# EasyVision-Ton/VMG

Measured on AMD Instinct MI355X. Metric: LR-frames/s (train: forward+loss+backward+AdamW), VMG-REDS-few_levels 4x SR, higher is better.
Workload: dtype bf16; 1 GPU; VMG-REDS-few_levels train step, per-GPU batch 4x7x3x64x64 -> 4x SR (BASELINE configs[1]); global_batch=4, frames_per_clip=7, parallelism=dp1, launch=eager, recompute_chains=False, fp8_chains=False

## Files before the change

include/vmg_hip.h:

```cpp
#ifndef VMG_HIP_H
#define VMG_HIP_H

#include <stdint.h>

#ifdef __cplusplus
extern "C" {
#endif

#define VMG_F32 0
#define VMG_BF16 1

#define VMG_ACT_NONE 0
#define VMG_ACT_RELU 1
#define VMG_ACT_LRELU 2
#define VMG_ACT_GELU 3

#define VMG_CONV_GENERAL 0
#define VMG_CONV_KSPLIT 2
#define VMG_CONV_WS 3
#define VMG_CONV_LINEAR_WRES 4
#define VMG_CONV_WSTAT 6

const char* vmg_last_error(void);
int vmg_version(void);

typedef struct vmg_ctx vmg_ctx;
vmg_ctx* vmg_create(int device);
int vmg_destroy(vmg_ctx* ctx);
int vmg_ctx_device(const vmg_ctx* ctx);
int vmg_max_lds_bytes(void);

int64_t vmg_conv_pack_bytes(int dtype, int ks, int on, int nsrc, const int* src_ch, int cout_tiles);
int vmg_conv_pack(int dtype, const float* w, int O, int I, int ks, int o0, int on, int nsrc, const int* src_off,
                  const int* src_ch, int transpose_flip, int cout_tiles, void* packed, void* stream);

int64_t vmg_convws_pack_bytes(int on, int nsrc, const int* src_ch, int cout_tiles);
int vmg_convws_pack(const float* w, int O, int I, int o0, int on, int nsrc, const int* src_off, const int* src_ch, int transpose_flip,
                    int cout_tiles, void* packed, void* stream);

typedef struct vmg_conv_desc {
  int dtype, ks, cout_tiles;
  int N, H, W, Cout;
  int nsrc;
  const void* src[4];
  int64_t src_ps[4];
  int src_ch[4];
  const void* packed;
  const float* bias;
  void* out;
  int64_t out_ps;
  void* out_pre;
  const void* res;
  int64_t res_ps;
  const void* aux;
  int64_t aux_ps;
  int act;
  float slope, alpha;
  int actgrad;
  int pixel_shuffle;
  int mt;
  int deep;
} vmg_conv_desc;

int vmg_conv_fwd(const vmg_conv_desc* d, void* stream);
enum {
  VMG_CONV_FAM_IGEMM = 1,
  VMG_CONV_FAM_KSPLIT = 2,
  VMG_CONV_FAM_WS = 3,
  VMG_CONV_FAM_LINEAR_WRES = 4,
  VMG_CONV_FAM_WSTAT = 5,
  VMG_CONV_PLAN_INTS = 11
};
int vmg_conv_fwd_plan(const vmg_conv_desc* d, int ncu, int* plan);
typedef struct vmg_chain_desc {
  int dtype, N, H, W, C, nblk, nsrc;
  const void* src[4];
  int64_t src_ps[4];
  int src_ch[4];
  const void* packed0;
  const float* bias0;
  float slope0;
  int cout_tiles0, deep0;
  const void* const* packed1;
  const float* const* bias1;
  const void* const* packed2;
  const float* const* bias2;
  float r_scaling;
  int cout_tiles, deep;
  void* const* y;
  void* const* t;
  void* const* g_y;
  void* const* g_t;
} vmg_chain_desc;
int vmg_resblock_chain_fwd(const vmg_chain_desc* d, void* stream);
int vmg_resblock_chain_bwd(const vmg_chain_desc* d, void* stream);

void* vmg_replay_build(void* hip_graph, int* n_ops, int* n_kernels);
int vmg_replay_kernel_info(void* replay, int idx, void** func, unsigned* grid_x, unsigned* block_x, void** first_arg);
int vmg_replay_run(void* replay, int first, int last, void* stream);
void vmg_replay_destroy(void* replay);

int vmg_pack_entry_bytes(void);
int vmg_pack_entry(void* entry, int kind, int dtype, const float* w, int O, int I, int ks, int o0, int on, int nsrc, const int* src_off,
// ... 280 lines not shown
```

vmg_amd/csrc/common.h:

```cpp
#pragma once
#include <hip/hip_runtime.h>
#include <stdint.h>
#include <stdio.h>
#include <string.h>

#include "../../include/vmg_hip.h"

typedef __bf16 bf16;
typedef __attribute__((ext_vector_type(8))) __bf16 bf16x8;
typedef __attribute__((ext_vector_type(4))) __bf16 bf16x4;
typedef __attribute__((ext_vector_type(4))) float f32x4;

#define LDS_PTR(p) ((__attribute__((address_space(3))) void*)(p))
#define GLB_PTR(p) ((const __attribute__((address_space(1))) void*)(p))

void vmg_set_error(const char* fmt, ...);

constexpr int VMG_MAX_DEVICES = 64;
int vmg_current_device();
int vmg_cu_count(int device);

bool vmg_prof_before(int klass, long long pixels, hipStream_t st);
void vmg_prof_after(hipStream_t st);
#define VMG_PROF_CONV3X3 1
// ... 30 lines not shown
  static constexpr int CHUNKB = 32;
};

__device__ __forceinline__ float to_f32(bf16 v) { return (float)v; }
__device__ __forceinline__ float to_f32(float v) { return v; }
template <typename T>
__device__ __forceinline__ T from_f32(float v);
template <>
__device__ __forceinline__ bf16 from_f32<bf16>(float v) { return (bf16)v; }
template <>
__device__ __forceinline__ float from_f32<float>(float v) { return v; }

__device__ __forceinline__ void load4(const bf16* p, float v[4]) {
  bf16x4 t = *reinterpret_cast<const bf16x4*>(p);
  v[0] = (float)t[0]; v[1] = (float)t[1]; v[2] = (float)t[2]; v[3] = (float)t[3];
}
__device__ __forceinline__ void load4(const float* p, float v[4]) {
  float4 t = *reinterpret_cast<const float4*>(p);
  v[0] = t.x; v[1] = t.y; v[2] = t.z; v[3] = t.w;
}
__device__ __forceinline__ void store4(bf16* p, const float v[4]) {
  bf16x4 t = {(bf16)v[0], (bf16)v[1], (bf16)v[2], (bf16)v[3]};
  *reinterpret_cast<bf16x4*>(p) = t;
}
__device__ __forceinline__ void store4(float* p, const float v[4]) {
  *reinterpret_cast<float4*>(p) = make_float4(v[0], v[1], v[2], v[3]);
}

__device__ __forceinline__ float gelu_erf(float x) { return 0.5f * x * (1.0f + erff(x * 0.70710678118654752440f)); }
__device__ __forceinline__ float gelu_erf_grad(float x) {
  return 0.5f * (1.0f + erff(x * 0.70710678118654752440f)) + x * __expf(-0.5f * x * x) * 0.39894228040143267794f;
}

__device__ __forceinline__ float wave_sum(float v) {
#pragma unroll
  for (int o = 32; o > 0; o >>= 1) v += __shfl_xor(v, o, 64);
  return v;
}
__device__ __forceinline__ float wave_max(float v) {
#pragma unroll
  for (int o = 32; o > 0; o >>= 1) v = fmaxf(v, __shfl_xor(v, o, 64));
  return v;
}

static inline int64_t cdiv64(int64_t a, int64_t b) { return (a + b - 1) / b; }
static inline int cdiv(int a, int b) { return (a + b - 1) / b; }
```

vmg_amd/csrc/conv_igemm.hip:

```cpp
#include <stdlib.h>

#include <type_traits>

#include "common.h"

namespace {

constexpr int MAX_ISRC = 32;
constexpr int CBMAX = 160;

__host__ __device__ constexpr int kstg(int ks) { return ks > 1 ? ks : 2; }
__host__ __device__ constexpr int stage_bytes(int ks, int ntb, int cb) { return kstg(ks) * 4 * ntb * 16 * cb; }
__host__ __device__ constexpr int stage_stride(int ks, int ntb, int cb) { return (stage_bytes(ks, ntb, cb) + 4095) / 4096 * 4096; }
__host__ __device__ inline int stages_of(int ks, int ch) {
  const int nb = (ch / 8 + 3) / 4;
  return ks > 1 ? ks * nb : (nb + 1) / 2;
}

struct ConvK {
  const char* src[MAX_ISRC];
  long long src_ps[MAX_ISRC];
  short src_ch[MAX_ISRC];
  short src_nst[MAX_ISRC];
  int src_pixb[MAX_ISRC];
// ... 410 lines not shown
  for (int mt = 0; mt < MT; ++mt) {
    f32x4 r[NTB];
#pragma unroll
    for (int ct = 0; ct < NTB; ++ct) r[ct] = acc[ct][mt];
    conv_epilogue_row<T, KS, NTB>(a, r, wave * MT + mt, TH, cb, nt_real, n, ty, tx, m0, px, g);
  }
}

template <int NTB>
struct EpiLds {
  static constexpr int COB = NTB * 16, C8 = 2 * NTB, PSTR = COB * 4 + 16, NIT = (16 * C8 + 63) / 64;
  static constexpr int BYTES = 16 * PSTR;
};

template <int KS, int NTB>
__device__ __forceinline__ void conv_epilogue_prefetch8(const ConvK& a, int row, int TH, int cb, int n, int ty, int tx, long long m0, int lane,
                                                        bf16x8 (&pre_res)[EpiLds<NTB>::NIT], bf16x8 (&pre_aux)[EpiLds<NTB>::NIT]) {
  using E = EpiLds<NTB>;
  const bf16* res = reinterpret_cast<const bf16*>(a.res);
  const bf16* aux = reinterpret_cast<const bf16*>(a.aux);
#pragma unroll
  for (int it = 0; it < E::NIT; ++it) {
    const int j = it * 64 + lane, pxi = j / E::C8, c8 = j - pxi * E::C8;
    long long pix;
    const bool valid = conv_row_pixel<KS>(a, row, TH, n, ty, tx, m0, pxi & 15, pix);
    const int co = cb * E::COB + c8 * 8;
    if (j < 16 * E::C8 && valid && co < a.Cout) {
      if (res) pre_res[it] = *reinterpret_cast<const bf16x8*>(res + pix * a.res_ps + co);
      if (aux) pre_aux[it] = *reinterpret_cast<const bf16x8*>(aux + pix * a.aux_ps + co);
    }
  }
}

template <int KS, int NTB>
__device__ __forceinline__ void conv_epilogue_lds8(const ConvK& a, const f32x4 (&acc)[NTB], char* stg, int row, int TH, int cb, int n, int ty, int tx,
                                                   long long m0, int lane, const bf16x8 (&pre_res)[EpiLds<NTB>::NIT],
                                                   const bf16x8 (&pre_aux)[EpiLds<NTB>::NIT], const float* lbias) {
  using E = EpiLds<NTB>;
  const int px = lane & 15, g = lane >> 4;
#pragma unroll
  for (int ct = 0; ct < NTB; ++ct) *reinterpret_cast<f32x4*>(stg + px * E::PSTR + (ct * 16 + g * 4) * 4) = acc[ct];
  bf16* out = reinterpret_cast<bf16*>(a.out);
  bf16* out_pre = reinterpret_cast<bf16*>(a.out_pre);
  const float neg = a.act == VMG_ACT_RELU ? 0.f : (a.act == VMG_ACT_LRELU ? a.slope : 1.f);
#pragma unroll
  for (int it = 0; it < E::NIT; ++it) {
    const int j = it * 64 + lane, pxi = j / E::C8, c8 = j - pxi * E::C8;
    long long pix;
    const bool valid = conv_row_pixel<KS>(a, row, TH, n, ty, tx, m0, pxi & 15, pix);
    const int co = cb * E::COB + c8 * 8;
    if (!(j < 16 * E::C8 && valid && co < a.Cout) || VMG_DBG(a, 8)) continue;
    const f32x4 lo = *reinterpret_cast<const f32x4*>(stg + pxi * E::PSTR + c8 * 32);
    const f32x4 hi = *reinterpret_cast<const f32x4*>(stg + pxi * E::PSTR + c8 * 32 + 16);
    float v[8] = {lo[0], lo[1], lo[2], lo[3], hi[0], hi[1], hi[2], hi[3]};
    if (a.bias) {
      const f32x4 b0 = *reinterpret_cast<const f32x4*>(lbias + c8 * 8), b1 = *reinterpret_cast<const f32x4*>(lbias + c8 * 8 + 4);
#pragma unroll
      for (int r = 0; r < 4; ++r) { v[r] += b0[r]; v[4 + r] += b1[r]; }
    }
    if (out_pre) {
      bf16x8 t;
#pragma unroll
      for (int r = 0; r < 8; ++r) t[r] = (bf16)v[r];
      *reinterpret_cast<bf16x8*>(out_pre + pix * a.out_ps + co) = t;
    }
    if (a.act == VMG_ACT_GELU) {
#pragma unroll
      for (int r = 0; r < 8; ++r) v[r] = gelu_erf(v[r]) * a.alpha;
    } else {
#pragma unroll
      for (int r = 0; r < 8; ++r) v[r] = (v[r] > 0.f ? v[r] : v[r] * neg) * a.alpha;
    }
    if (a.aux) {
#pragma unroll
      for (int r = 0; r < 8; ++r) {
        const float u = (float)pre_aux[it][r];
        v[r] *= a.actgrad == 3 ? gelu_erf_grad(u) : (u > 0.f ? 1.f : (a.actgrad == 2 ? a.slope : 0.f));
      }
    }
    if (a.res) {
#pragma unroll
      for (int r = 0; r < 8; ++r) v[r] += (float)pre_res[it][r];
    }
    bf16x8 t;
#pragma unroll
    for (int r = 0; r < 8; ++r) t[r] = (bf16)v[r];
    *reinterpret_cast<bf16x8*>(out + pix * a.out_ps + co) = t;
  }
}

template <typename T, int KS, int NTB>
__global__ __launch_bounds__(256, (NTB <= 3 ? 3 : 2)) void conv_ksplit_kernel(const ConvK a) {
  constexpr int ES = ElemTraits<T>::ES, CB = ElemTraits<T>::CHUNKB;
  constexpr int TH = 4;
  constexpr int TWH = 16 + KS - 1;
  constexpr int COB = NTB * 16;
  constexpr int SS = stage_stride(KS, NTB, CB);
  constexpr int KSB = 4 * COB * CB;
  extern __shared__ __attribute__((aligned(16))) char smem[];
  char* halo = smem;
  char* zslot = smem + a.halo_bytes;
  float* lbias = reinterpret_cast<float*>(zslot + 16);
  if (VMG_DBG(a, 16)) return;

  const int tid = threadIdx.x, lane = tid & 63;
  const int wave = __builtin_amdgcn_readfirstlane(tid >> 6);
  const int px = lane & 15, g = lane >> 4;
  const int cb = blockIdx.y;
  const int nt_real = min(NTB, (a.Cout - cb * COB + 15) >> 4);
  int n = 0, ty = 0, tx = 0;
// ... 210 lines not shown
    }
  };
  int boff[NK];
#pragma unroll
  for (int k = 0; k < NK; ++k) {
    const int sb = k / NKS, kk = k - sb * NKS;
    boff[k] = px * pixb + (sb * CH + min(4 * kk + g, CH - 1)) * CB;
  }

  issue(t0, 0);
  int buf = 0;
  for (int t = t0; t < t1; ++t, buf ^= 1) {
    const long long m0 = (long long)t * 16;
    bf16x8 pre_res[EpiLds<NTB>::NIT], pre_aux[EpiLds<NTB>::NIT];
    conv_epilogue_prefetch8<KS, NTB>(a, 0, 4, cb, 0, 0, 0, m0, lane, pre_res, pre_aux);
    if (t + 1 < t1) {
      issue(t + 1, buf ^ 1);
      asm volatile("s_waitcnt vmcnt(%0)" ::"n"(NDMA) : "memory");
    } else {
      asm volatile("s_waitcnt vmcnt(0)" ::: "memory");
    }
    f32x4 acc[NTB];
#pragma unroll
    for (int ct = 0; ct < NTB; ++ct) acc[ct] = f32x4{0.f, 0.f, 0.f, 0.f};
    const char* xb = xbuf + buf * XBUF;
#pragma unroll
    for (int k = 0; k < NK; ++k) {
      Frag<T> xf;
      xf.load(xb + boff[k]);
#pragma unroll
      for (int ct = 0; ct < NTB; ++ct) acc[ct] = mma(wres[k][ct], xf, acc[ct]);
    }
    conv_epilogue_lds8<KS, NTB>(a, acc, patch, 0, 4, cb, 0, 0, 0, m0, lane, pre_res, pre_aux, a.bias ? a.bias + cb * COB : nullptr);
  }
}

template <int NCT, int NB, bool FULL>
__global__ __launch_bounds__(512, 1) void conv_wstat_kernel(const ConvK a, int ntiles) {
  using T = bf16;
  constexpr int KS = 3, CB = 16, TH = 8, TWH = 18, THH = 10;
  constexpr int COB = NCT * 16, KSB = 4 * COB * CB;
  constexpr int SS = stage_stride(KS, NCT, CB);
  constexpr int NK = 9 * NB, RW = NCT < 2 ? NCT : 2;
  constexpr int PIXB = 144;
  constexpr int HVEC = THH * TWH * 9, NDMA = (HVEC + 63) / 64, HB = NDMA * 1024;
  constexpr int PSTR = COB * 4 + 16, C8 = 2 * NCT, NITEM = 128 * C8;
  extern __shared__ __attribute__((aligned(16))) char smem[];
  const int tid = threadIdx.x, lane = tid & 63;
  const int wave = __builtin_amdgcn_readfirstlane(tid >> 6);
  const int px = lane & 15, g = lane >> 4;
  const int cb = blockIdx.y;
  const int CH = a.src_ch[0] >> 3;
  constexpr int wbytes = 3 * NB * SS;
  char* wl = smem;
  char* halo = smem + wbytes;
  float* lbias = reinterpret_cast<float*>(halo + 2 * HB);
  char* patch = halo + 2 * HB + COB * 4;

  const int per_xcd = gridDim.x >> 3;
  const int xcd = blockIdx.x & 7, local = blockIdx.x >> 3;
  const int band = (ntiles + 7) >> 3;
  const int band0 = xcd * band, band1 = min(ntiles, band0 + band);
  auto tile_of = [&](int it) { return band0 + it * per_xcd + local; };
  auto barrier = [&]() {
    asm volatile("s_waitcnt lgkmcnt(0)" ::: "memory");
    __builtin_amdgcn_s_barrier();
// ... 829 lines not shown

int choose_pixb(int ch, int es, int cb) {
  static const int grp[4][16] = {{0, 1, 2, 3, 12, 13, 14, 15, 20, 21, 22, 23, 24, 25, 26, 27},
                                 {4, 5, 6, 7, 8, 9, 10, 11, 16, 17, 18, 19, 28, 29, 30, 31},
                                 {32, 33, 34, 35, 44, 45, 46, 47, 52, 53, 54, 55, 56, 57, 58, 59},
                                 {36, 37, 38, 39, 40, 41, 42, 43, 48, 49, 50, 51, 60, 61, 62, 63}};
  int best = ch * es, bestc = 1 << 30;
  for (int pad = 0; pad <= 240; pad += 16) {
    const int pixb = ch * es + pad;
    int worst = 0;
    for (int gi = 0; gi < 4; ++gi) {
      int cnt[16] = {0};
      for (int j = 0; j < 16; ++j) {
        const int l = grp[gi][j];
        const int addr = (l & 15) * pixb + (l >> 4) * cb;
        int c = ++cnt[(addr >> 4) & 15];
        if (c > worst) worst = c;
      }
    }
    if (worst < bestc) { bestc = worst; best = pixb; }
    if (worst == 1) break;
  }
  return best;
}

struct ConvPlan {
  int family;
  int dtype, ks, mt, ntb;
  int variant;
  int vec8;
  int gx, gy;
  int tpw;
  int lds;
};

constexpr int epi_lds_bytes(int ntb) { return 16 * (ntb * 16 * 4 + 16); }
constexpr int wres_lds_bytes(int ntb, int ns) { return 4 * (2 * 5 * ns * 1024 + ((epi_lds_bytes(ntb) + 1023) & ~1023)); }
constexpr int wstat_lds_bytes(int nct, int nb) {
  return 3 * nb * stage_stride(3, nct, 16) + 2 * (((10 * 18 * 9 + 63) / 64) * 1024) + nct * 16 * 4 + 128 * (nct * 64 + 16);
}
constexpr int ws_stage_bytes(int nct) { return 3 * nct * 16 * 64; }

template <typename T, int KS, int MT, int NTB>
int launch_conv(const ConvK& k, const ConvPlan& p, hipStream_t st) {
  const int lds = p.lds;
  auto fn = conv_igemm_kernel<T, KS, MT, NTB>;
  static bool attr_set[VMG_MAX_DEVICES] = {};
  const int dev = vmg_current_device();
  if (!attr_set[dev]) {
    (void)hipFuncSetAttribute(reinterpret_cast<const void*>(fn), hipFuncAttributeMaxDynamicSharedMemorySize, 160 * 1024);
    attr_set[dev] = true;
  }
  const bool prof = (KS == 3 && sizeof(T) == 2 && k.nsrc == 1 && k.src_ch[0] == 144 && k.Cout == 144) && vmg_prof_before(VMG_PROF_CONV3X3, k.M, st);
  hipLaunchKernelGGL(fn, dim3((unsigned)p.gx, p.gy), dim3(256), lds, st, k);
  if (prof) vmg_prof_after(st);
  VMG_LAUNCH_CHECK();
  return 0;
}

template <typename T, int KS, int MT>
int dispatch_ntb(const ConvK& k, const ConvPlan& p, hipStream_t st) {
  switch (p.ntb) {
    case 1: return launch_conv<T, KS, MT, 1>(k, p, st);
    case 3: return launch_conv<T, KS, MT, 3>(k, p, st);
    case 4: return launch_conv<T, KS, MT, 4>(k, p, st);
    case 5: return launch_conv<T, KS, MT, 5>(k, p, st);
    case 7: return launch_conv<T, KS, MT, 7>(k, p, st);
    case 8: return launch_conv<T, KS, MT, 8>(k, p, st);
    case 9: return launch_conv<T, KS, MT, 9>(k, p, st);
  }
  vmg_set_error("conv: cout_tiles must be 1, 3, 4, 5, 7, 8 or 9 (got %d)", p.ntb);
  return -1;
}

// ... 22 lines not shown
  hipLaunchKernelGGL(fn, dim3((unsigned)p.gx, p.gy), dim3(256), lds, st, k);
  if (prof) vmg_prof_after(st);
  VMG_LAUNCH_CHECK();
  return 0;
}

template <typename T, int KS>
int dispatch_ksplit(const ConvK& k, const ConvPlan& p, hipStream_t st) {
  switch (p.ntb) {
    case 1: return launch_ksplit<T, KS, 1>(k, p, st);
    case 3: return launch_ksplit<T, KS, 3>(k, p, st);
    case 4: return launch_ksplit<T, KS, 4>(k, p, st);
    case 5: return launch_ksplit<T, KS, 5>(k, p, st);
  }
  vmg_set_error("conv (k-split): cout_tiles must be 1, 3, 4 or 5 (got %d)", p.ntb);
  return -1;
}

template <int NTB, int NS = 1>
int launch_linear_wres(const ConvK& k, const ConvPlan& p, hipStream_t st) {
  static_assert(wres_lds_bytes(NTB, NS) == 4 * (2 * 5 * NS * 1024 + ((EpiLds<NTB>::BYTES + 1023) & ~1023)), "linear_wres_kernel: LDS");
  const int lds = p.lds;
  auto fn = linear_wres_kernel<NTB, NS>;
  static bool attr_set[VMG_MAX_DEVICES] = {};
  const int dev = vmg_current_device();
  if (!attr_set[dev]) {
    (void)hipFuncSetAttribute(reinterpret_cast<const void*>(fn), hipFuncAttributeMaxDynamicSharedMemorySize, 160 * 1024);
    attr_set[dev] = true;
  }
  hipLaunchKernelGGL(fn, dim3((unsigned)p.gx, p.gy), dim3(256), lds, st, k, (int)cdiv64(k.M, 16), p.tpw);
  VMG_LAUNCH_CHECK();
  return 0;
}

template <int NCT, int NB, bool FULL>
int launch_wstat2(const ConvK& k, const ConvPlan& p, hipStream_t st) {
  constexpr int lds = wstat_lds_bytes(NCT, NB);
  static_assert(lds <= 160 * 1024, "conv_wstat_kernel: LDS");
  auto fn = conv_wstat_kernel<NCT, NB, FULL>;
  static bool attr_set[VMG_MAX_DEVICES] = {};
  const int dev = vmg_current_device();
  if (!attr_set[dev]) {
    (void)hipFuncSetAttribute(reinterpret_cast<const void*>(fn), hipFuncAttributeMaxDynamicSharedMemorySize, 160 * 1024);
    attr_set[dev] = true;
  }
  hipLaunchKernelGGL(fn, dim3((unsigned)p.gx, p.gy), dim3(512), lds, st, k, (int)((long long)k.N * k.tiles_y * k.tiles_x));
  VMG_LAUNCH_CHECK();
  return 0;
}

template <int NCT, int NB>
int launch_wstat(const ConvK& k, const ConvPlan& p, hipStream_t st) {
  return (p.variant >> 4) ? launch_wstat2<NCT, NB, true>(k, p, st) : launch_wstat2<NCT, NB, false>(k, p, st);
}

template <int NCT>
int launch_ws(const ConvK& k, const ConvPlan& p, hipStream_t st) {
  using G = WsGeo<NCT>;
  static_assert(ws_stage_bytes(NCT) == G::STG, "conv_ws_kernel: stage bytes");
  const int lds = p.lds;
  auto fn = conv_ws_kernel<NCT>;
  static bool attr_set[VMG_MAX_DEVICES] = {};
  const int dev = vmg_current_device();
  if (!attr_set[dev]) {
    (void)hipFuncSetAttribute(reinterpret_cast<const void*>(fn), hipFuncAttributeMaxDynamicSharedMemorySize, 160 * 1024);
    attr_set[dev] = true;
// ... 171 lines not shown
  int rc;
  if (kind == 1) {
    VMG_CHECK(ks == 3 && dtype == VMG_BF16, "pack_entry: the weight-streaming layout is bf16 3x3");
    rc = fill_pack_ws(e.p, e.total, w, O, I, o0, on, nsrc, src_off, src_ch, transpose_flip, cout_tiles, packed);
  } else {
    rc = fill_pack_std(e.p, e.total, dtype, w, O, I, ks, o0, on, nsrc, src_off, src_ch, transpose_flip, cout_tiles, packed);
  }
  if (rc) return rc;
  e.kind = kind; e.dtype = dtype; e.blk0 = blk0;
  long long nb = e.p.fast3 ? (e.p.units + 255) / 256 : (e.total + 256LL * 16 - 1) / (256LL * 16);
  e.nblk = (int)(nb < 1 ? 1 : (nb > 64 ? 64 : nb));
  memcpy(entry, &e, sizeof(e));
  return e.nblk;
}

extern "C" int vmg_pack_run(const void* plan_dev, int n, int total_blocks, void* stream) {
  VMG_CHECK(plan_dev && n > 0 && total_blocks > 0, "pack_run: bad arguments");
  static_assert(sizeof(PackEntry) % 4 == 0, "the block-owner table sits behind the entries");
  hipLaunchKernelGGL(pack_batch_kernel, dim3(total_blocks), dim3(256), 0, (hipStream_t)stream, (const PackEntry*)plan_dev, n);
  VMG_LAUNCH_CHECK();
  return 0;
}

static int conv_plan(const vmg_conv_desc* d, int ncu, ConvK& k, ConvPlan& p) {
  VMG_CHECK(d != nullptr, "conv_fwd: null descriptor");
  VMG_CHECK(d->ks == 1 || d->ks == 3 || d->ks == 7, "conv_fwd: ks must be 1, 3 or 7");
  VMG_CHECK(d->dtype == VMG_F32 || d->dtype == VMG_BF16, "conv_fwd: bad dtype");
  VMG_CHECK(d->nsrc >= 1 && d->nsrc <= 4, "conv_fwd: nsrc must be 1..4");
  VMG_CHECK(d->N > 0 && d->H > 0 && d->W > 0 && d->Cout > 0, "conv_fwd: bad shape");
  VMG_CHECK(d->packed && d->out, "conv_fwd: null packed weights / output");
  VMG_CHECK(!d->pixel_shuffle || (d->Cout % 4 == 0), "conv_fwd: pixel_shuffle needs Cout %% 4 == 0");
  VMG_CHECK(!(d->actgrad != 0 && d->aux == nullptr), "conv_fwd: actgrad without aux");
  VMG_CHECK(d->deep == VMG_CONV_GENERAL || d->deep == VMG_CONV_KSPLIT || d->deep == VMG_CONV_WS || d->deep == VMG_CONV_LINEAR_WRES ||
                d->deep == VMG_CONV_WSTAT,
            "conv_fwd: unknown kernel route deep = %d", d->deep);
  const int es = d->dtype == VMG_BF16 ? 2 : 4, cbytes = es * 8;
  memset(&k, 0, sizeof(k));
  memset(&p, 0, sizeof(p));
  short xoff[MAX_ISRC];
  int parent[MAX_ISRC];
  const int n = expand_sources(d->nsrc, nullptr, d->src_ch, xoff, k.src_ch, parent);
  VMG_CHECK(n > 0, "conv_fwd: source channel counts must be multiples of 8");
  int mt = d->mt;
  if (d->dtype == VMG_F32) mt = 1;
  const long long M = (long long)d->N * d->H * d->W;
  const int ntb = d->cout_tiles;
  VMG_CHECK(ntb > 0, "conv_fwd: cout_tiles must be positive");
  const int ncb = cdiv(d->Cout, ntb * 16);
  if (d->ks == 7) mt = 1;
  if (mt == 0) mt = 1;
  VMG_CHECK(mt == 1 || mt == 2, "conv_fwd: mt must be 1 or 2");
  const int TH = 4 * mt, TWH = 16 + d->ks - 1, THH = TH + d->ks - 1;
  int kt = 0, halo = 0;
  for (int s = 0; s < n; ++s) {
    const int par = parent[s];
    VMG_CHECK(d->src[par] != nullptr, "conv_fwd: null source %d", par);
    VMG_CHECK(d->src_ps[par] >= d->src_ch[par] && (d->src_ps[par] * es) % 16 == 0, "conv_fwd: source pixel stride must be >= channels and 16-byte aligned");
    VMG_CHECK(((uintptr_t)d->src[par]) % 16 == 0, "conv_fwd: source pointer must be 16-byte aligned");
    k.src[s] = (const char*)d->src[par] + (long long)xoff[s] * es;
    k.src_ps[s] = d->src_ps[par];
    k.src_nst[s] = (short)stages_of(d->ks, k.src_ch[s]);
    k.src_pixb[s] = choose_pixb(k.src_ch[s], es, cbytes);
    kt += k.src_nst[s];
    const int hb = THH * TWH * k.src_pixb[s];
    if (hb > halo) halo = hb;
  }
  k.nsrc = n;
// ... 26 lines not shown
    int kt3 = 0, halo3 = 0;
    for (int s = 0; s < n; ++s) {
      k.src_pixb[s] = k.src_ch[s] * 2;
      k.src_nst[s] = (short)(ws_ksteps(k.src_ch[s] >> 3) / 3);
      kt3 += k.src_nst[s];
      const int hb = 10 * 18 * k.src_pixb[s];
      if (hb > halo3) halo3 = hb;
    }
    k.nstages = kt3;
    k.halo_bytes = (halo3 + 1023) & ~1023;
    k.tiles_y = cdiv(d->H, 8);
    k.ring = ntb <= 3 ? 3 : ((k.halo_bytes + 4 * ws_stage_bytes(ntb) + ntb * 16 * 4 <= 160 * 1024) ? 4 : 3);
    p.lds = k.halo_bytes + k.ring * ws_stage_bytes(ntb) + ntb * 16 * 4;
    VMG_CHECK(p.lds <= 160 * 1024, "conv (weight-streaming): LDS request %d B exceeds 160 KiB", p.lds);
    const long long nblk = (long long)k.N * k.tiles_y * k.tiles_x;
    VMG_CHECK(nblk > 0 && nblk < (1ll << 31), "conv: bad grid %lld", nblk);
    p.family = VMG_CONV_FAM_WS; p.gx = (int)nblk;
    return 0;
  }
  if (d->deep == VMG_CONV_WSTAT && d->dtype == VMG_BF16 && d->ks == 3 && mt == 1 && k.vec8 && n == 1 && (ntb == 1 || ntb == 3 || ntb == 4) && k.src_ch[0] <= 64 && k.src_ch[0] % 8 == 0 &&
      k.src_ps[0] % 8 == 0 && d->W <= 255 * 16 && (long long)d->W * k.src_ps[0] * 2 * 10 < (1ll << 31)) {
    const int nb = (k.src_ch[0] / 8 + 3) / 4;
    VMG_CHECK(k.nstages == 3 * nb, "conv (weights-stationary): %d stages in the pack, %d expected", k.nstages, 3 * nb);
    k.tiles_y = cdiv(d->H, 8);
    const long long ntiles = (long long)k.N * k.tiles_y * k.tiles_x;
    VMG_CHECK(ntiles > 0 && ntiles < (1ll << 30), "conv: bad tile count %lld", ntiles);
    int nwg = cus() & ~7;
    if (nwg < 8) nwg = 8;
    while (nwg > 8 && (long long)(nwg >> 3) > cdiv64(ntiles, 8)) nwg -= 8;
    const bool full = k.res || k.aux || k.out_pre || k.act == VMG_ACT_GELU;
    p.family = VMG_CONV_FAM_WSTAT; p.variant = nb | (full ? 16 : 0); p.gx = nwg; p.lds = wstat_lds_bytes(ntb, nb);
    return 0;
  }
  if (d->deep == VMG_CONV_LINEAR_WRES && d->dtype == VMG_BF16 && d->ks == 1 && k.vec8 && (ntb == 3 || ntb == 5)) {
    int ns = 0;
    if (n == 1 && k.src_ch[0] <= 160 && k.src_pixb[0] == k.src_ch[0] * 2) ns = 1;
    else if (n == 2 && ntb == 3 && d->nsrc == 1 && k.src_ch[0] == k.src_ch[1] && k.src_ch[0] <= 160 && k.src[1] == k.src[0] + k.src_ch[0] * 2 &&
             k.src_nst[0] == k.src_nst[1])
      ns = 2;
    if (ns) {
      const long long ntiles = cdiv64(k.M, 16);
      VMG_CHECK(ntiles > 0 && ntiles < (1ll << 31), "conv: bad tile count %lld", ntiles);
      const int wg_per_cu = ns == 1 ? 2 : 1, c = cus();
      long long waves = (long long)(wg_per_cu * c / ncb > 0 ? wg_per_cu * c / ncb : 1) * 4;
      long long tpw = cdiv64(ntiles, waves);
      if (tpw < 4) tpw = 4;
      p.family = VMG_CONV_FAM_LINEAR_WRES; p.variant = ns; p.gx = (int)cdiv64(cdiv64(ntiles, tpw), 4); p.tpw = (int)tpw; p.lds = wres_lds_bytes(ntb, ns);
      return 0;
    }
  }
  const bool ksplit = d->ks != 7 && d->deep == VMG_CONV_KSPLIT;
  if (ksplit) {
    VMG_CHECK(d->dtype == VMG_BF16 && mt == 1, "conv_fwd: the k-split variant is bf16, mt = 1");
    if (!(ntb == 1 || ntb == 3 || ntb == 4 || ntb == 5)) {
      vmg_set_error("conv (k-split): cout_tiles must be 1, 3, 4 or 5 (got %d)", ntb);
      return -1;
    }
    const int scratch = 12 * ntb * 1024;
    p.lds = (k.halo_bytes > scratch ? k.halo_bytes : scratch) + 16 + ntb * 16 * 4;
    VMG_CHECK(p.lds <= 160 * 1024, "conv (k-split): LDS request %d B exceeds 160 KiB", p.lds);
    k.halo_bytes = p.lds - 16 - ntb * 16 * 4;
    p.family = VMG_CONV_FAM_KSPLIT;
  } else {
    if (d->ks == 7) {
      if (!(ntb == 1 || ntb == 2 || ntb == 4)) {
        vmg_set_error("conv (7x7): cout_tiles must be 1, 2 or 4 (got %d)", ntb);
        return -1;
      }
    } else if (!(ntb == 1 || ntb == 3 || ntb == 4 || ntb == 5 || ntb == 7 || ntb == 8 || ntb == 9)) {
      vmg_set_error("conv: cout_tiles must be 1, 3, 4, 5, 7, 8 or 9 (got %d)", ntb);
      return -1;
    }
    p.lds = k.halo_bytes + 2 * stage_stride(d->ks, ntb, cbytes);
    VMG_CHECK(p.lds <= 160 * 1024, "conv: LDS request %d B exceeds 160 KiB", p.lds);
    p.family = VMG_CONV_FAM_IGEMM;
  }
  const long long nblk = (d->ks > 1) ? (long long)k.N * k.tiles_y * k.tiles_x : cdiv64(k.M, 64 * mt);
  VMG_CHECK(nblk > 0 && nblk < (1ll << 31), "conv: bad grid %lld", nblk);
  p.gx = (int)nblk;
  return 0;
}

static int conv_launch(const ConvK& k, const ConvPlan& p, hipStream_t st) {
  switch (p.family) {
    case VMG_CONV_FAM_WS:
      return p.ntb == 9 ? launch_ws<9>(k, p, st) : (p.ntb == 7 ? launch_ws<7>(k, p, st) : (p.ntb == 8 ? launch_ws<8>(k, p, st) : launch_ws<3>(k, p, st)));
    case VMG_CONV_FAM_WSTAT:
      switch (p.ntb * 2 + ((p.variant & 15) - 1)) {
        case 2: return launch_wstat<1, 1>(k, p, st);
        case 3: return launch_wstat<1, 2>(k, p, st);
        case 6: return launch_wstat<3, 1>(k, p, st);
        case 7: return launch_wstat<3, 2>(k, p, st);
        case 8: return launch_wstat<4, 1>(k, p, st);
        case 9: return launch_wstat<4, 2>(k, p, st);
      }
      break;
    case VMG_CONV_FAM_LINEAR_WRES:
      if (p.variant == 2) return launch_linear_wres<3, 2>(k, p, st);
      return p.ntb == 3 ? launch_linear_wres<3>(k, p, st) : launch_linear_wres<5>(k, p, st);
    case VMG_CONV_FAM_KSPLIT:
      return p.ks == 3 ? dispatch_ksplit<bf16, 3>(k, p, st) : dispatch_ksplit<bf16, 1>(k, p, st);
    case VMG_CONV_FAM_IGEMM:
      if (p.ks == 7) return p.dtype == VMG_BF16 ? dispatch_ks7<bf16>(k, p, st) : dispatch_ks7<float>(k, p, st);
      if (p.dtype == VMG_BF16) {
        if (p.ks == 3) return p.mt == 2 ? dispatch_ntb<bf16, 3, 2>(k, p, st) : dispatch_ntb<bf16, 3, 1>(k, p, st);
        return p.mt == 2 ? dispatch_ntb<bf16, 1, 2>(k, p, st) : dispatch_ntb<bf16, 1, 1>(k, p, st);
      }
      if (p.ks == 3) return dispatch_ntb<float, 3, 1>(k, p, st);
      return dispatch_ntb<float, 1, 1>(k, p, st);
  }
  vmg_set_error("conv_fwd: no kernel for plan family %d", p.family);
  return -1;
}

extern "C" int vmg_conv_fwd(const vmg_conv_desc* d, void* stream) {
  ConvK k;
  ConvPlan p;
  if (conv_plan(d, 0, k, p)) return -1;
  return conv_launch(k, p, (hipStream_t)stream);
}

extern "C" int vmg_conv_fwd_plan(const vmg_conv_desc* d, int ncu, int* plan) {
  VMG_CHECK(plan != nullptr && ncu >= 0, "conv_fwd_plan: null plan / negative ncu");
  ConvK k;
  ConvPlan p;
  if (conv_plan(d, ncu, k, p)) return -1;
  const int v[VMG_CONV_PLAN_INTS] = {p.family, p.dtype, p.ks, p.mt, p.ntb, p.variant, p.vec8, p.gx, p.gy, p.tpw, p.lds};
  for (int i = 0; i < VMG_CONV_PLAN_INTS; ++i) plan[i] = v[i];
  return 0;
}

static void chain_base(const vmg_chain_desc* c, vmg_conv_desc& d) {
// ... 44 lines not shown
```

vmg_amd/functional.py:

```python
from __future__ import annotations

import contextlib
from typing import List, Optional, Sequence

import torch

from . import hip
from . import kernels as K
from .hip import HipError
from .wgrad import DEFERRED, _wgrad_entries, _wgrad_now, flush_deferred_wgrads, recorded, set_wgrad_mode

class _Fn(torch.autograd.Function):

    @classmethod
    def apply(cls, *args):
        return super(torch.autograd.Function, cls).apply(*args)


def _pad_to(n: int, m: int = 8) -> int:
    return (n + m - 1) // m * m


def choose_tiling(M: int, cout: int, ks: int, dtype: torch.dtype, src_ch: Optional[Sequence[int]] = None, pixel_shuffle: bool = False):
    if USE_WS and src_ch is not None and not pixel_shuffle:
        t = K.ws_eligible(cout, ks, dtype, src_ch)
        if t and M <= 16384 and cout in (112, 144):
            return (4 if cout == 112 else 3), 1, hip.CONV_KSPLIT
        if t:
            return t, 1, hip.CONV_WS
    if dtype == torch.bfloat16 and ks == 3 and cout in (144, 288):
        return 3, 1, hip.CONV_KSPLIT
    if dtype == torch.bfloat16 and ks == 1 and src_ch is not None and len(src_ch) == 1 and M >= 65536 and not pixel_shuffle:
        if cout == 144 and src_ch[0] == 144:
            return 5, 1, hip.CONV_LINEAR_WRES
        if cout == 288 and src_ch[0] == 144:
            return 5, 1, hip.CONV_LINEAR_WRES
        if cout == 144 and src_ch[0] == 288:
            return 3, 1, hip.CONV_LINEAR_WRES
    if dtype == torch.bfloat16 and ks == 3 and not pixel_shuffle and M >= (1 << 18) and src_ch is not None and len(src_ch) == 1 and \
            src_ch[0] <= 64 and src_ch[0] % 8 == 0 and cout in (16, 48, 64):
        return cout // 16, 1, hip.CONV_WSTAT
    if dtype == torch.bfloat16 and ks == 3 and not pixel_shuffle and M >= (1 << 20) and src_ch is not None and len(src_ch) == 1 and \
            (cout <= 16 or src_ch[0] <= 16):
        return None, 2, hip.CONV_GENERAL
    return None, 1, hip.CONV_GENERAL


USE_WS = True
GROUPED_DENSE = True

class _PlanState:

    def __init__(self):
        self.plan, self.stamp, self.wkey, self.ents, self.packs = K.PackPlan(), -1, None, [], []


def _from_param(ent) -> bool:
    pw, weight = ent[1], ent[2]
    return pw.call is not None and pw.call[0] == weight.data_ptr()


class _PackCache:

    def __init__(self):
        self.ents = {}
        self.q8 = {}
        self.volatile = set()
        self.epoch = 0
        self.stamp = 0
        self.stable = _PlanState()
        self.vol = _PlanState()
        self.decay = None

    def get(self, key, weight: torch.Tensor, build, planned: bool = True):
        ents = self.ents if planned else self.q8
        ver = (weight._version, self.epoch)
        hit = ents.get(key)
        buf = None
        if hit is not None:
            if hit[2] is weight:
# ... 1565 lines not shown
```

vmg_amd/hip.py:

```python
from __future__ import annotations

import ctypes
import os
from ctypes import POINTER, c_char_p, c_float, c_int, c_int64, c_void_p

import torch

HERE = os.path.dirname(os.path.abspath(__file__))
LIB_PATH = os.environ.get("VMG_HIP_LIB") or os.path.join(HERE, "libvmg_hip.so")

F32, BF16 = 0, 1
ACT_NONE, ACT_RELU, ACT_LRELU, ACT_GELU = 0, 1, 2, 3
GATE_ACTS = {"tanh": 0, "sigmoid": 1, "relu": 2, "gelu": 3, "swish": 4}
SHIFT_VECTOR, SHIFT_ELEMENT = 1, 2
DWCONV_VECTOR, DWCONV_ELEMENT, DWCONV_PLAN_INTS = 1, 2, 8
CONV_GENERAL, CONV_KSPLIT, CONV_WS, CONV_LINEAR_WRES, CONV_WSTAT = 0, 2, 3, 4, 6
CONV_FAM_IGEMM, CONV_FAM_KSPLIT, CONV_FAM_WS, CONV_FAM_LINEAR_WRES, CONV_FAM_WSTAT = 1, 2, 3, 4, 5
CONV_PLAN_INTS = 11
MORPHFC_PLAN_INTS = 8
MORPH_ROUTE_ELEMENT, MORPH_ROUTE_LDS = 0, 1
WGRAD_V1, WGRAD_3, WGRAD_3B, WGRAD_L2, WGRAD_7 = 1, 2, 3, 4, 5


def wgrad_kernel_id(kind: int, a: int = 0, b: int = 0, c: int = 0) -> int:
    return kind << 24 | a << 16 | b << 8 | c


class HipError(RuntimeError):
    pass


class ConvDesc(ctypes.Structure):
    _fields_ = [
        ("dtype", c_int), ("ks", c_int), ("cout_tiles", c_int),
        ("N", c_int), ("H", c_int), ("W", c_int), ("Cout", c_int),
        ("nsrc", c_int),
        ("src", c_void_p * 4), ("src_ps", c_int64 * 4), ("src_ch", c_int * 4),
        ("packed", c_void_p), ("bias", c_void_p),
        ("out", c_void_p), ("out_ps", c_int64), ("out_pre", c_void_p),
        ("res", c_void_p), ("res_ps", c_int64),
        ("aux", c_void_p), ("aux_ps", c_int64),
        ("act", c_int), ("slope", c_float), ("alpha", c_float),
        ("actgrad", c_int), ("pixel_shuffle", c_int), ("mt", c_int), ("deep", c_int),
    ]


class ChainDesc(ctypes.Structure):
    _fields_ = [
        ("dtype", c_int), ("N", c_int), ("H", c_int), ("W", c_int), ("C", c_int), ("nblk", c_int), ("nsrc", c_int),
        ("src", c_void_p * 4), ("src_ps", c_int64 * 4), ("src_ch", c_int * 4),
# ... 262 lines not shown
```

vmg_amd/kernels.py:

```python
from __future__ import annotations

import collections
import ctypes
import os
import struct
from typing import Optional, Sequence, Tuple

import torch

from . import hip
from .hip import ConvDesc, HipError


def _intarr(v: Sequence[int]):
    return (ctypes.c_int * len(v))(*[int(x) for x in v])


def cout_tiles_for(cout: int, dtype: torch.dtype = torch.bfloat16, ks: int = 3) -> int:
    t = (cout + 15) // 16
    if t <= 1:
        return 1
    if ks == 7:
        return 2 if t == 2 else 4
    if t <= 4:
        return 4
    best, waste = None, None
    for cand in ((5, 4) if dtype == torch.float32 else (9, 8, 7, 5)):
        w = (t + cand - 1) // cand * cand - t
        if waste is None or w < waste:
            best, waste = cand, w
    return best


class PackedConv:

    __slots__ = ("buf", "dtype", "ks", "cout", "src_ch", "cout_tiles", "layout", "call")

    def __init__(self, buf, dtype, ks, cout, src_ch, cout_tiles, layout="std", call=None):
        self.buf, self.dtype, self.ks, self.cout, self.src_ch, self.cout_tiles = buf, dtype, ks, cout, list(src_ch), cout_tiles
        self.layout = layout
        self.call = call


def pack_conv_weight(w: torch.Tensor, dtype: torch.dtype, src_ch: Optional[Sequence[int]] = None,
                     src_off: Optional[Sequence[int]] = None, o0: int = 0, on: Optional[int] = None,
                     transpose_flip: bool = False, out: Optional[torch.Tensor] = None, cout_tiles: Optional[int] = None, groups: int = 1) -> PackedConv:
    hip.require_cuda(w)
    if w.dtype != torch.float32 or not w.is_contiguous():
        raise HipError("pack_conv_weight expects a contiguous fp32 weight")
    if w.dim() == 2:
        O, I, ks = w.shape[0], w.shape[1], 1
    elif w.dim() == 4 and w.shape[2] == w.shape[3]:
        O, I, ks = w.shape[0], w.shape[1], w.shape[2]
    else:
        raise HipError(f"unsupported weight shape {tuple(w.shape)}")
    kdim, odim = (O, I * groups) if transpose_flip else (I * groups, O)
    if src_ch is None:
        src_ch, src_off = [kdim], [0]
    if src_off is None:
        src_off, acc = [], 0
        for c in src_ch:
            src_off.append(acc)
            acc += c
    if on is None:
# ... 1788 lines not shown
```

Baseline: 578.8 LR-frames/s.

## Add persistent LDS-resident-weight linear rows kernel for 1x1 bf16 convs

Adds a new 1x1 conv (linear) kernel that loads the whole packed weight matrix into LDS once per block. Each wave then streams over its assigned 16-row tiles, prefetching the next tile's inputs and fusing the bias, activation-gradient and residual epilogue. It is routed for a few channel shapes (288->144, 192->192, 224->224) with large row counts, so weight reloads and launch-grid overhead are paid once per block. The cost is a single block per CU with large LDS use, a fixed set of template instances, and a separate GELU-grad variant with FP contraction disabled.

```diff
diff --git a/include/vmg_hip.h b/include/vmg_hip.h
--- a/include/vmg_hip.h
+++ b/include/vmg_hip.h
@@ -20,6 +20,7 @@
 #define VMG_CONV_WS 3
 #define VMG_CONV_LINEAR_WRES 4
 #define VMG_CONV_WSTAT 6
+enum { VMG_CONV_LINEAR_ROWS = 8 };
 
 const char* vmg_last_error(void);
 int vmg_version(void);
@@ -69,6 +70,7 @@
   VMG_CONV_FAM_WS = 3,
   VMG_CONV_FAM_LINEAR_WRES = 4,
   VMG_CONV_FAM_WSTAT = 5,
+  VMG_CONV_FAM_LINEAR_ROWS = 6,
   VMG_CONV_PLAN_INTS = 11
 };
 int vmg_conv_fwd_plan(const vmg_conv_desc* d, int ncu, int* plan);
diff --git a/vmg_amd/csrc/common.h b/vmg_amd/csrc/common.h
--- a/vmg_amd/csrc/common.h
+++ b/vmg_amd/csrc/common.h
@@ -86,6 +86,13 @@
   return 0.5f * (1.0f + erff(x * 0.70710678118654752440f)) + x * __expf(-0.5f * x * x) * 0.39894228040143267794f;
 }
 
+__device__ __forceinline__ float gelu_erf_grad_sep(float x) {
+#pragma clang fp contract(off)
+  const float h = 0.5f * (1.0f + erff(x * 0.70710678118654752440f));
+  const float t = x * __expf(-0.5f * x * x) * 0.39894228040143267794f;
+  return h + t;
+}
+
 __device__ __forceinline__ float wave_sum(float v) {
 #pragma unroll
   for (int o = 32; o > 0; o >>= 1) v += __shfl_xor(v, o, 64);
diff --git a/vmg_amd/csrc/conv_igemm.hip b/vmg_amd/csrc/conv_igemm.hip
--- a/vmg_amd/csrc/conv_igemm.hip
+++ b/vmg_amd/csrc/conv_igemm.hip
@@ -466,7 +466,7 @@
   }
 }
 
-template <int KS, int NTB>
+template <int KS, int NTB, bool SEP = false>
 __device__ __forceinline__ void conv_epilogue_lds8(const ConvK& a, const f32x4 (&acc)[NTB], char* stg, int row, int TH, int cb, int n, int ty, int tx,
                                                    long long m0, int lane, const bf16x8 (&pre_res)[EpiLds<NTB>::NIT],
                                                    const bf16x8 (&pre_aux)[EpiLds<NTB>::NIT], const float* lbias) {
@@ -509,7 +509,7 @@
 #pragma unroll
       for (int r = 0; r < 8; ++r) {
         const float u = (float)pre_aux[it][r];
-        v[r] *= a.actgrad == 3 ? gelu_erf_grad(u) : (u > 0.f ? 1.f : (a.actgrad == 2 ? a.slope : 0.f));
+        v[r] *= a.actgrad == 3 ? (SEP ? gelu_erf_grad_sep(u) : gelu_erf_grad(u)) : (u > 0.f ? 1.f : (a.actgrad == 2 ? a.slope : 0.f));
       }
     }
     if (a.res) {
@@ -786,6 +786,92 @@
       for (int ct = 0; ct < NTB; ++ct) acc[ct] = mma(wres[k][ct], xf, acc[ct]);
     }
     conv_epilogue_lds8<KS, NTB>(a, acc, patch, 0, 4, cb, 0, 0, 0, m0, lane, pre_res, pre_aux, a.bias ? a.bias + cb * COB : nullptr);
+  }
+}
+
+template <int NKS, int NS, int NTB, int NCB>
+__global__ __launch_bounds__(512, 1) void linear_rows_kernel(const ConvK a, int ntiles, int tiles_per_wave) {
+  using T = bf16;
+  constexpr int KS = 1, CB = 16, NK = NKS * NS;
+  constexpr int COB = NTB * 16;
+  constexpr int SS = stage_stride(KS, NTB, CB);
+  constexpr int KSB = 4 * COB * CB;
+  constexpr int NST = (NKS + 1) / 2;
+  constexpr int NV = NCB * NK * (KSB / 16);
+  constexpr int PATCH = (EpiLds<NTB>::BYTES + 1023) & ~1023;
+  constexpr int NIT = EpiLds<NTB>::NIT;
+  extern __shared__ __attribute__((aligned(16))) char smem[];
+  const int tid = threadIdx.x, lane = tid & 63, nthr = blockDim.x;
+  const int wave = __builtin_amdgcn_readfirstlane(tid >> 6);
+  const int px = lane & 15, g = lane >> 4;
+  const int CH = a.src_ch[0] >> 3;
+  const long long ps_b = a.src_ps[0] * 2;
+  const int t0 = (blockIdx.x * (nthr >> 6) + wave) * tiles_per_wave, t1 = min(ntiles, t0 + tiles_per_wave);
+
+  int coff[NK];
+#pragma unroll
+  for (int k = 0; k < NK; ++k) {
+    const int sb = k / NKS, kk = k - sb * NKS;
+    coff[k] = (sb * CH + min(4 * kk + g, CH - 1)) * CB;
+  }
+  auto load_x = [&](int t, bf16x8 (&x)[NK]) {
+    const long long row = (long long)t * 16 + px;
+    const bool ok = t < t1 && row < a.M;
+    const char* rp = a.src[0] + row * ps_b;
+#pragma unroll
+    for (int k = 0; k < NK; ++k) x[k] = *reinterpret_cast<const bf16x8*>(ok ? rp + coff[k] : reinterpret_cast<const char*>(&g_conv_zero16));
+  };
+  bf16x8 xc[NK], xn[NK];
+  load_x(t0, xc);
+
+  {
+    constexpr int WB = 8;
+    for (int v0 = tid; v0 < NV; v0 += nthr * WB) {
+      uint4 r[WB];
+#pragma unroll
+      for (int j = 0; j < WB; ++j) {
+        const int v = min(v0 + j * nthr, NV - 1);
+        const int ck = v / (KSB / 16), rem = v - ck * (KSB / 16);
+        const int cb = ck / NK, k = ck - cb * NK;
+        const int sb = k / NKS, kk = k - sb * NKS;
+        r[j] = *reinterpret_cast<const uint4*>(a.wpack + (long long)(cb * (NS * NST) + sb * NST + (kk >> 1)) * SS + (kk & 1) * KSB + rem * 16);
+      }
+#pragma unroll
+      for (int j = 0; j < WB; ++j)
+        if (v0 + j * nthr < NV) *reinterpret_cast<uint4*>(smem + (v0 + j * nthr) * 16) = r[j];
+    }
+  }
+  __syncthreads();
+  if (t0 >= t1) return;
+
+  const char* wl = smem + g * (COB * CB) + px * CB;
+  char* patch = smem + NV * 16 + wave * PATCH;
+  for (int t = t0; t < t1; ++t) {
+    const long long m0 = (long long)t * 16;
+    bf16x8 pre_res[NCB][NIT], pre_aux[NCB][NIT];
+#pragma unroll
+    for (int cb = 0; cb < NCB; ++cb) conv_epilogue_prefetch8<KS, NTB>(a, 0, 4, cb, 0, 0, 0, m0, lane, pre_res[cb], pre_aux[cb]);
+    load_x(t + 1, xn);
+#pragma unroll
+    for (int cb = 0; cb < NCB; ++cb) {
+      f32x4 acc[NTB];
+#pragma unroll
+      for (int ct = 0; ct < NTB; ++ct) acc[ct] = f32x4{0.f, 0.f, 0.f, 0.f};
+#pragma unroll
+      for (int k = 0; k < NK; ++k) {
+        Frag<T> xf;
+        xf.v = xc[k];
+#pragma unroll
+        for (int ct = 0; ct < NTB; ++ct) {
+          Frag<T> wf;
+          wf.load(wl + (cb * NK + k) * KSB + ct * 16 * CB);
+          acc[ct] = mma(wf, xf, acc[ct]);
+        }
+      }
+      conv_epilogue_lds8<KS, NTB, true>(a, acc, patch, 0, 4, cb, 0, 0, 0, m0, lane, pre_res[cb], pre_aux[cb], a.bias ? a.bias + cb * COB : nullptr);
+    }
+#pragma unroll
+    for (int k = 0; k < NK; ++k) xc[k] = xn[k];
   }
 }
 
@@ -1681,6 +1767,7 @@
   int gx, gy;
   int tpw;
   int lds;
+  int nw;
 };
 
 constexpr int epi_lds_bytes(int ntb) { return 16 * (ntb * 16 * 4 + 16); }
@@ -1689,6 +1776,8 @@
   return 3 * nb * stage_stride(3, nct, 16) + 2 * (((10 * 18 * 9 + 63) / 64) * 1024) + nct * 16 * 4 + 128 * (nct * 64 + 16);
 }
 constexpr int ws_stage_bytes(int nct) { return 3 * nct * 16 * 64; }
+constexpr int rows_weight_bytes(int nk, int ntb, int ncb) { return ncb * nk * 4 * ntb * 16 * 16; }
+constexpr int rows_patch_bytes(int ntb) { return (epi_lds_bytes(ntb) + 1023) & ~1023; }
 
 template <typename T, int KS, int MT, int NTB>
 int launch_conv(const ConvK& k, const ConvPlan& p, hipStream_t st) {
@@ -1777,6 +1866,24 @@
   VMG_LAUNCH_CHECK();
   return 0;
 }
+
+template <int NKS, int NS, int NTB, int NCB>
+int launch_linear_rows(const ConvK& k, const ConvPlan& p, hipStream_t st) {
+  static_assert(rows_patch_bytes(NTB) == ((EpiLds<NTB>::BYTES + 1023) & ~1023), "linear_rows_kernel: patch");
+  static_assert(rows_weight_bytes(NKS * NS, NTB, NCB) + 4 * rows_patch_bytes(NTB) <= 160 * 1024, "linear_rows_kernel: LDS");
+  auto fn = linear_rows_kernel<NKS, NS, NTB, NCB>;
+  static bool attr_set[VMG_MAX_DEVICES] = {};
+  const int dev = vmg_current_device();
+  if (!attr_set[dev]) {
+    (void)hipFuncSetAttribute(reinterpret_cast<const void*>(fn), hipFuncAttributeMaxDynamicSharedMemorySize, 160 * 1024);
+    attr_set[dev] = true;
+  }
+  hipLaunchKernelGGL(fn, dim3((unsigned)p.gx, 1), dim3(64 * p.nw), p.lds, st, k, (int)cdiv64(k.M, 16), p.tpw);
+  VMG_LAUNCH_CHECK();
+  return 0;
+}
+
+constexpr int ROWS_INSTANCES[5][4] = {{5, 1, 9, 1}, {5, 1, 9, 2}, {5, 2, 9, 1}, {3, 2, 4, 3}, {4, 2, 7, 2}};
 
 template <int NCT, int NB, bool FULL>
 int launch_wstat2(const ConvK& k, const ConvPlan& p, hipStream_t st) {
@@ -2014,7 +2121,7 @@
   VMG_CHECK(!d->pixel_shuffle || (d->Cout % 4 == 0), "conv_fwd: pixel_shuffle needs Cout %% 4 == 0");
   VMG_CHECK(!(d->actgrad != 0 && d->aux == nullptr), "conv_fwd: actgrad without aux");
   VMG_CHECK(d->deep == VMG_CONV_GENERAL || d->deep == VMG_CONV_KSPLIT || d->deep == VMG_CONV_WS || d->deep == VMG_CONV_LINEAR_WRES ||
-                d->deep == VMG_CONV_WSTAT,
+                d->deep == VMG_CONV_WSTAT || d->deep == VMG_CONV_LINEAR_ROWS,
             "conv_fwd: unknown kernel route deep = %d", d->deep);
   const int es = d->dtype == VMG_BF16 ? 2 : 4, cbytes = es * 8;
   memset(&k, 0, sizeof(k));
@@ -2107,6 +2214,27 @@
     p.family = VMG_CONV_FAM_WSTAT; p.variant = nb | (full ? 16 : 0); p.gx = nwg; p.lds = wstat_lds_bytes(ntb, nb);
     return 0;
   }
+  if (d->deep == VMG_CONV_LINEAR_ROWS && d->dtype == VMG_BF16 && d->ks == 1 && k.vec8 && d->nsrc == 1 && d->src_ch[0] % 16 == 0 && d->src_ch[0] <= 320 &&
+      d->Cout <= 320 && d->Cout == ncb * ntb * 16 && (n == 1 || n == 2) && k.src_ps[0] * 2 * 16 < (1ll << 31)) {
+    const int nks = (k.src_ch[0] / 8 + 3) / 4;
+    bool have = false;
+    for (const auto& inst : ROWS_INSTANCES) have = have || (inst[0] == nks && inst[1] == n && inst[2] == ntb && inst[3] == ncb);
+    const int wbytes = rows_weight_bytes(nks * n, ntb, ncb), patch = rows_patch_bytes(ntb);
+    int nwmax = (160 * 1024 - wbytes) / patch;
+    if (nwmax > 8) nwmax = 8;
+    const long long ntiles = cdiv64(k.M, 16);
+    if (have && nwmax >= 4 && ntiles < (1ll << 30)) {
+      VMG_CHECK(k.nstages == n * ((nks + 1) / 2), "conv (linear rows): %d stages in the pack, %d expected", k.nstages, n * ((nks + 1) / 2));
+      const int c = cus();
+      const long long tpw = cdiv64(ntiles, (long long)c * nwmax);
+      const long long waves = cdiv64(ntiles, tpw);
+      int nw = (int)cdiv64(waves, c);
+      if (nw < 4) nw = 4;
+      p.family = VMG_CONV_FAM_LINEAR_ROWS; p.variant = ncb; p.gx = (int)cdiv64(waves, nw); p.gy = 1; p.tpw = (int)tpw; p.nw = nw;
+      p.lds = wbytes + nw * patch;
+      return 0;
+    }
+  }
   if (d->deep == VMG_CONV_LINEAR_WRES && d->dtype == VMG_BF16 && d->ks == 1 && k.vec8 && (ntb == 3 || ntb == 5)) {
     int ns = 0;
     if (n == 1 && k.src_ch[0] <= 160 && k.src_pixb[0] == k.src_ch[0] * 2) ns = 1;
@@ -2173,6 +2301,11 @@
     case VMG_CONV_FAM_LINEAR_WRES:
       if (p.variant == 2) return launch_linear_wres<3, 2>(k, p, st);
       return p.ntb == 3 ? launch_linear_wres<3>(k, p, st) : launch_linear_wres<5>(k, p, st);
+    case VMG_CONV_FAM_LINEAR_ROWS:
+      if (p.ntb == 4) return launch_linear_rows<3, 2, 4, 3>(k, p, st);
+      if (p.ntb == 7) return launch_linear_rows<4, 2, 7, 2>(k, p, st);
+      if (p.variant == 2) return launch_linear_rows<5, 1, 9, 2>(k, p, st);
+      return k.nsrc == 2 ? launch_linear_rows<5, 2, 9, 1>(k, p, st) : launch_linear_rows<5, 1, 9, 1>(k, p, st);
     case VMG_CONV_FAM_KSPLIT:
       return p.ks == 3 ? dispatch_ksplit<bf16, 3>(k, p, st) : dispatch_ksplit<bf16, 1>(k, p, st);
     case VMG_CONV_FAM_IGEMM:
diff --git a/vmg_amd/functional.py b/vmg_amd/functional.py
--- a/vmg_amd/functional.py
+++ b/vmg_amd/functional.py
@@ -30,7 +30,9 @@
             return t, 1, hip.CONV_WS
     if dtype == torch.bfloat16 and ks == 3 and cout in (144, 288):
         return 3, 1, hip.CONV_KSPLIT
-    if dtype == torch.bfloat16 and ks == 1 and src_ch is not None and len(src_ch) == 1 and M >= 65536 and not pixel_shuffle:
+    if dtype == torch.bfloat16 and ks == 1 and src_ch is not None and len(src_ch) == 1 and M >= LINEAR_MIN_ROWS and not pixel_shuffle:
+        if (src_ch[0], cout) in LINEAR_ROWS_SHAPES:
+            return K.linear_rows_tiles(src_ch[0], cout), 1, hip.CONV_LINEAR_ROWS
         if cout == 144 and src_ch[0] == 144:
             return 5, 1, hip.CONV_LINEAR_WRES
         if cout == 288 and src_ch[0] == 144:
@@ -46,6 +48,8 @@
     return None, 1, hip.CONV_GENERAL
 
 
+LINEAR_MIN_ROWS = 65536
+LINEAR_ROWS_SHAPES = {(288, 144), (192, 192), (224, 224)}
 USE_WS = True
 GROUPED_DENSE = True
 
diff --git a/vmg_amd/hip.py b/vmg_amd/hip.py
--- a/vmg_amd/hip.py
+++ b/vmg_amd/hip.py
@@ -16,6 +16,7 @@
 DWCONV_VECTOR, DWCONV_ELEMENT, DWCONV_PLAN_INTS = 1, 2, 8
 CONV_GENERAL, CONV_KSPLIT, CONV_WS, CONV_LINEAR_WRES, CONV_WSTAT = 0, 2, 3, 4, 6
 CONV_FAM_IGEMM, CONV_FAM_KSPLIT, CONV_FAM_WS, CONV_FAM_LINEAR_WRES, CONV_FAM_WSTAT = 1, 2, 3, 4, 5
+CONV_LINEAR_ROWS, CONV_FAM_LINEAR_ROWS = 8, 6
 CONV_PLAN_INTS = 11
 MORPHFC_PLAN_INTS = 8
 MORPH_ROUTE_ELEMENT, MORPH_ROUTE_LDS = 0, 1
diff --git a/vmg_amd/kernels.py b/vmg_amd/kernels.py
--- a/vmg_amd/kernels.py
+++ b/vmg_amd/kernels.py
@@ -30,6 +30,13 @@
         if waste is None or w < waste:
             best, waste = cand, w
     return best
+
+
+_LINEAR_ROWS_TILES = {(144, 144): 9, (144, 288): 9, (288, 144): 9, (192, 192): 4, (224, 224): 7}
+
+
+def linear_rows_tiles(cin: int, cout: int) -> int:
+    return _LINEAR_ROWS_TILES.get((cin, cout), 0)
 
 
 class PackedConv:
```

Result: slower. 460.0 LR-frames/s (-20.5%).
